# ANRGUSC/DEFER

Hardware: AMD Instinct MI355X
Metric: images/sec (whole node) ResNet50 pipeline (higher is better)
Workload: dtype bf16; 1 GPU; model=resnet50, global_batch=256, micro_batch=256, input=224x224x3 NHWC, parallelism=pp1, compression=none, hip_graphs=False, dual_rail=False, weights=random-init

## Files before the change

defer_amd/csrc/bindings.cpp:

```cpp
#include <torch/extension.h>
#include <ATen/hip/HIPContext.h>

#include <cstdlib>
#include <functional>
#include <mutex>
#include <string>
#include <unordered_map>

#include "kernels.h"

namespace {

using at::Tensor;
using defer_hip::ConvParams;

hipStream_t cur_stream() {
    return at::cuda::getCurrentHIPStream().stream();
}

const void* bptr(const Tensor& t) { return t.data_ptr(); }
void* bptr_mut(Tensor& t) { return t.data_ptr(); }

void check_bf16(const Tensor& t, const char* name) {
    TORCH_CHECK(t.is_cuda(), name, " must be on GPU");
// ... 377 lines not shown
    int64_t max_blocks) {
    check_bf16(x, "x");
    check_bf16(w3, "w3");
    check_bf16(w1, "w1");
    check_bf16(res, "res");
    TORCH_CHECK(x.dim() == 4 && w3.dim() == 4 && w1.dim() == 4 &&
                w3.size(1) == 1 && w3.size(2) == 1 && w1.size(1) == 1 &&
                w1.size(2) == 1, "conv1x1_chain wants NHWC x, 1x1 weights");
    TORCH_CHECK(mode >= 0 && mode <= 2, "mode must be 0, 1 or 2");
    int NB = x.size(0), H = x.size(1), W = x.size(2), K1 = x.size(3);
    int N1 = w3.size(0), N2 = w1.size(0);
    TORCH_CHECK(w3.size(3) == K1 && w1.size(3) == N1, "channel mismatch");
    TORCH_CHECK(res.dim() == 4 && res.size(0) == NB && res.size(1) == H &&
                res.size(2) == W && res.size(3) == N1,
                "res must match the expand output");
    TORCH_CHECK((!s3 || s3->numel() == N1) && (!b3 || b3->numel() == N1) &&
                (!s1 || s1->numel() == N2) && (!b1 || b1->numel() == N2),
                "scale/bias length must equal the conv's Cout");
    long M = (long)NB * H * W;
    TORCH_CHECK(M < (1LL << 31), "M too large");
    if (mode != 2 && K1 % 64 == 0 && N1 % 64 == 0 && N2 % 64 == 0) {
        auto y = at::empty({NB, H, W, N1}, x.options());
        auto a2 = at::empty({NB, H, W, N2}, x.options());
        if (defer_hip::launch_conv1x1_chain(
                bptr(x), bptr(w3), fptr_opt(s3, "s3", ones_buf(), N1),
                fptr_opt(b3, "b3", zeros_buf(), N1), bptr(res),
                bptr_mut(y), relu3, bptr(w1),
                fptr_opt(s1, "s1", ones_buf(), N2),
                fptr_opt(b1, "b1", zeros_buf(), N2), bptr_mut(a2), relu1,
                (int)M, K1, N1, N2, mode == 1, (int)max_blocks,
                cur_stream()))
            return {y, a2};
    }
    auto y = conv2d_bn_act(x, w3, s3, b3, res, 1, 0, relu3);
    auto a2 = conv2d_bn_act(y, w1, s1, b1, c10::nullopt, 1, 0, relu1);
    return {y, a2};
}

Tensor bn_act(Tensor x, Tensor scale, Tensor bias, bool relu) {
    if (is_f32(x, "x")) {
        check_f32(x, "x");
        int C = x.size(-1);
        TORCH_CHECK(C % 4 == 0, "fp32 bn_act needs C % 4 == 0, got ", C);
        TORCH_CHECK(scale.is_cuda() && bias.is_cuda() &&
                    scale.numel() == C && bias.numel() == C,
                    "scale/bias must be GPU tensors of length C");
        auto out = at::empty_like(x);
        auto sf = scale.to(at::kFloat).contiguous();
        auto bf = bias.to(at::kFloat).contiguous();
        defer_hip::launch_bn_act_f32(f32ptr(x), f32ptr(sf), f32ptr(bf),
                                     out.data_ptr<float>(), x.numel() / 4,
                                     C / 4, relu, cur_stream());
        return out;
    }
    check_bf16(x, "x");
    int C = x.size(-1);
    TORCH_CHECK(C % 8 == 0, "C must be a multiple of 8");
    auto out = at::empty_like(x);
    auto sf = scale.to(at::kFloat).contiguous();
    auto bf = bias.to(at::kFloat).contiguous();
    defer_hip::launch_bn_act(bptr(x), sf.data_ptr<float>(),
                             bf.data_ptr<float>(), bptr_mut(out),
                             x.numel() / 8, C / 8, relu, cur_stream());
    return out;
}

Tensor add_act(Tensor a, Tensor b, bool relu) {
    if (is_f32(a, "a")) {
        check_f32(a, "a");
        check_f32(b, "b");
        TORCH_CHECK(a.sizes() == b.sizes(), "shape mismatch");
        TORCH_CHECK(a.numel() % 4 == 0,
                    "fp32 add_act needs numel % 4 == 0");
        auto out = at::empty_like(a);
        defer_hip::launch_add_act_f32(f32ptr(a), f32ptr(b),
                                      out.data_ptr<float>(), a.numel() / 4,
                                      relu, cur_stream());
        return out;
    }
    check_bf16(a, "a");
    check_bf16(b, "b");
    TORCH_CHECK(a.sizes() == b.sizes(), "shape mismatch");
    TORCH_CHECK(a.numel() % 8 == 0, "numel must be a multiple of 8");
    auto out = at::empty_like(a);
    defer_hip::launch_add_act(bptr(a), bptr(b), bptr_mut(out),
                              a.numel() / 8, relu, cur_stream());
    return out;
}

Tensor relu(Tensor x) {
    if (is_f32(x, "x")) {
        check_f32(x, "x");
        TORCH_CHECK(x.numel() % 4 == 0, "fp32 relu needs numel % 4 == 0");
        auto out = at::empty_like(x);
        defer_hip::launch_relu_f32(f32ptr(x), out.data_ptr<float>(),
                                   x.numel() / 4, cur_stream());
        return out;
    }
    check_bf16(x, "x");
    TORCH_CHECK(x.numel() % 8 == 0, "numel must be a multiple of 8");
    auto out = at::empty_like(x);
    defer_hip::launch_relu(bptr(x), bptr_mut(out), x.numel() / 8,
                           cur_stream());
    return out;
}

Tensor softmax(Tensor x) {
    if (is_f32(x, "x")) {
        check_f32(x, "x");
        TORCH_CHECK(x.dim() >= 1 && x.numel() > 0, "softmax of nothing");
        int cols = x.size(-1);
        long rows = x.numel() / cols;
        auto out = at::empty_like(x);
        defer_hip::launch_softmax_f32(f32ptr(x), out.data_ptr<float>(),
                                      (int)rows, cols, cur_stream());
        return out;
    }
    check_bf16(x, "x");
    int cols = x.size(-1);
    long rows = x.numel() / cols;
    auto out = at::empty_like(x);
    defer_hip::launch_softmax(bptr(x), bptr_mut(out), (int)rows, cols,
                              cur_stream());
    return out;
}

Tensor maxpool2d(Tensor x, int64_t kernel, int64_t stride, int64_t pad) {
    if (is_f32(x, "x")) {
        check_f32(x, "x");
        TORCH_CHECK(x.dim() == 4, "x must be NHWC");
        int NB = x.size(0), H = x.size(1), W = x.size(2), C = x.size(3);
        TORCH_CHECK(C % 4 == 0, "fp32 maxpool2d needs C % 4 == 0, got ", C);
        int OH = (int)((H + 2 * pad - kernel) / stride + 1);
        int OW = (int)((W + 2 * pad - kernel) / stride + 1);
        auto out = at::empty({NB, OH, OW, C}, x.options());
        defer_hip::launch_maxpool_f32(f32ptr(x), out.data_ptr<float>(), NB, H,
                                 W, C, OH, OW, (int)kernel, (int)stride,
                                 (int)pad, cur_stream());
        return out;
    }
    check_bf16(x, "x");
    TORCH_CHECK(x.dim() == 4, "x must be NHWC");
    int NB = x.size(0), H = x.size(1), W = x.size(2), C = x.size(3);
    TORCH_CHECK(C % 8 == 0, "C must be a multiple of 8");
    int OH = (int)((H + 2 * pad - kernel) / stride + 1);
    int OW = (int)((W + 2 * pad - kernel) / stride + 1);
    auto out = at::empty({NB, OH, OW, C}, x.options());
    defer_hip::launch_maxpool(bptr(x), bptr_mut(out), NB, H, W, C, OH, OW,
                              (int)kernel, (int)stride, (int)pad,
                              cur_stream());
    return out;
}

Tensor avgpool2d(Tensor x, int64_t kernel, int64_t stride, int64_t pad) {
    if (is_f32(x, "x")) {
        check_f32(x, "x");
        TORCH_CHECK(x.dim() == 4, "x must be NHWC");
        int NB = x.size(0), H = x.size(1), W = x.size(2), C = x.size(3);
        TORCH_CHECK(C % 4 == 0, "fp32 avgpool2d needs C % 4 == 0, got ", C);
        int OH = (int)((H + 2 * pad - kernel) / stride + 1);
        int OW = (int)((W + 2 * pad - kernel) / stride + 1);
        auto out = at::empty({NB, OH, OW, C}, x.options());
        defer_hip::launch_avgpool_f32(f32ptr(x), out.data_ptr<float>(), NB, H,
                                 W, C, OH, OW, (int)kernel, (int)stride,
                                 (int)pad, cur_stream());
        return out;
    }
    check_bf16(x, "x");
    TORCH_CHECK(x.dim() == 4, "x must be NHWC");
    int NB = x.size(0), H = x.size(1), W = x.size(2), C = x.size(3);
    TORCH_CHECK(C % 8 == 0, "C must be a multiple of 8");
    int OH = (int)((H + 2 * pad - kernel) / stride + 1);
    int OW = (int)((W + 2 * pad - kernel) / stride + 1);
    auto out = at::empty({NB, OH, OW, C}, x.options());
    defer_hip::launch_avgpool(bptr(x), bptr_mut(out), NB, H, W, C, OH,
                              OW, (int)kernel, (int)stride, (int)pad,
                              cur_stream());
    return out;
}

Tensor concat_lastdim(std::vector<Tensor> xs) {
    TORCH_CHECK(!xs.empty(), "concat of nothing");
    auto base = xs[0].sizes().vec();
    int nd = (int)base.size();
    long rows = 1;
    for (int i = 0; i + 1 < nd; ++i) rows *= base[i];
    long ctot = 0;
    const bool f32 = is_f32(xs[0], "concat input");
    for (auto& t : xs) {
        if (f32) check_f32(t, "concat input");
        else check_bf16(t, "concat input");
        TORCH_CHECK((int)t.sizes().size() == nd, "rank mismatch");
        for (int i = 0; i + 1 < nd; ++i)
            TORCH_CHECK(t.size(i) == base[i], "leading-dim mismatch");
        ctot += t.size(nd - 1);
    }
    base[nd - 1] = ctot;
    auto out = at::empty(base, xs[0].options());
    hipStream_t s = cur_stream();
    if (f32) {
        if (xs.size() == 2 && xs[0].size(nd - 1) % 4 == 0 &&
            xs[1].size(nd - 1) % 4 == 0) {
            defer_hip::launch_cat2_f32(f32ptr(xs[0]), f32ptr(xs[1]),
                                       out.data_ptr<float>(), rows,
                                       (int)xs[0].size(nd - 1),
                                       (int)xs[1].size(nd - 1), s);
            return out;
        }
        long coff = 0;
        for (auto& t : xs) {
            long cj = t.size(nd - 1);
            hipMemcpy2DAsync((char*)bptr_mut(out) + coff * 4, ctot * 4,
                             bptr(t), cj * 4, cj * 4, rows,
                             hipMemcpyDeviceToDevice, s);
            coff += cj;
        }
        return out;
    }
    if (xs.size() == 2 && xs[0].size(nd - 1) % 8 == 0 &&
        xs[1].size(nd - 1) % 8 == 0) {
        defer_hip::launch_cat2(bptr(xs[0]), bptr(xs[1]), bptr_mut(out),
                               rows, (int)xs[0].size(nd - 1),
                               (int)xs[1].size(nd - 1), s);
        return out;
    }
    long coff = 0;
    for (auto& t : xs) {
        long cj = t.size(nd - 1);
        hipMemcpy2DAsync((char*)bptr_mut(out) + coff * 2, ctot * 2,
                         bptr(t), cj * 2, cj * 2, rows,
                         hipMemcpyDeviceToDevice, s);
        coff += cj;
    }
    return out;
}

Tensor global_avg_pool(Tensor x) {
    if (is_f32(x, "x")) {
        check_f32(x, "x");
        TORCH_CHECK(x.dim() == 4, "x must be NHWC");
        int NB = x.size(0), HW = x.size(1) * x.size(2), C = x.size(3);
        TORCH_CHECK(C % 4 == 0,
                    "fp32 global_avg_pool needs C % 4 == 0, got ", C);
        TORCH_CHECK(HW > 0, "empty spatial extent");
        auto out = at::empty({NB, C}, x.options());
        defer_hip::launch_gap_f32(f32ptr(x), out.data_ptr<float>(), NB, HW,
                                  C, cur_stream());
        return out;
    }
    check_bf16(x, "x");
    TORCH_CHECK(x.dim() == 4, "x must be NHWC");
    int NB = x.size(0), HW = x.size(1) * x.size(2), C = x.size(3);
    TORCH_CHECK(C % 8 == 0, "C must be a multiple of 8");
    auto out = at::empty({NB, C}, x.options());
    defer_hip::launch_gap(bptr(x), bptr_mut(out), NB, HW, C, cur_stream());
    return out;
}

std::tuple<int64_t, int64_t, int64_t> field_shape(const Tensor& t) {
    auto sz = t.sizes();
    int nd = sz.size();
    if (nd == 1) return {1, 1, sz[0]};
    if (nd == 2) return {1, sz[0], sz[1]};
    int64_t d0 = 1;
    for (int i = 0; i + 2 < nd; ++i) d0 *= sz[i];
    return {d0, sz[nd - 2], sz[nd - 1]};
}

Tensor zfp_encode(Tensor x, int64_t rate, c10::optional<Tensor> out,
                  int64_t phases = 3) {
    TORCH_CHECK(x.is_cuda() && x.is_contiguous(), "x must be GPU contig");
    bool bf16 = x.scalar_type() == at::kBFloat16;
    TORCH_CHECK(bf16 || x.scalar_type() == at::kFloat, "bf16/f32 only");
    auto [d0, d1, d2] = field_shape(x);
    long nb = ((d0 + 3) / 4) * ((d1 + 3) / 4) * ((d2 + 3) / 4);
    long bytes = nb * rate * 8;
    Tensor o;
    if (out) {
        TORCH_CHECK(out->numel() == bytes && out->is_contiguous()
                    && out->scalar_type() == at::kByte, "bad out buffer");
        o = *out;
    } else {
        o = at::empty({bytes},
                      x.options().dtype(at::kByte));
    }
    defer_hip::launch_zfp_encode(bptr(x), bptr_mut(o), bf16, (int)d0,
                                 (int)d1, (int)d2, (int)rate,
                                 cur_stream(), (int)phases);
    return o;
}

Tensor zfp_decode(Tensor wire, std::vector<int64_t> shape, int64_t rate,
                  bool bf16_out) {
    TORCH_CHECK(wire.is_cuda() && wire.is_contiguous()
                && wire.scalar_type() == at::kByte, "bad wire");
    auto o = at::empty(shape, wire.options().dtype(
                                  bf16_out ? at::kBFloat16 : at::kFloat));
    auto [d0, d1, d2] = field_shape(o);
    defer_hip::launch_zfp_decode(bptr(wire), bptr_mut(o), bf16_out,
                                 (int)d0, (int)d1, (int)d2, (int)rate,
                                 cur_stream());
    return o;
}

void fp8_encode(Tensor x, Tensor out) {
    check_bf16(x, "x");
    long n = x.numel();
    TORCH_CHECK(out.is_cuda() && out.is_contiguous()
                && out.scalar_type() == at::kByte
                && out.numel() == n + 4, "bad fp8 wire buffer");
    defer_hip::launch_fp8_encode(bptr(x), n, bptr_mut(out),
                                 cur_stream());
}

Tensor fp8_decode(Tensor wire, std::vector<int64_t> shape) {
    TORCH_CHECK(wire.is_cuda() && wire.is_contiguous()
                && wire.scalar_type() == at::kByte, "bad wire");
    auto y = at::empty(shape, wire.options().dtype(at::kBFloat16));
    TORCH_CHECK(y.numel() + 4 == wire.numel(), "wire/shape mismatch");
    defer_hip::launch_fp8_decode(bptr(wire), y.numel(), bptr_mut(y),
                                 cur_stream());
    return y;
}

Tensor lz4_compress(Tensor x) {
    TORCH_CHECK(x.is_cuda() && x.is_contiguous()
                && x.scalar_type() == at::kByte, "x must be GPU u8 contig");
    long n = x.numel();
    TORCH_CHECK(n > 0, "empty input");
    auto scratch = at::empty({defer_hip::lz4_scratch_bytes(n)},
                             x.options());
    auto o = at::empty({defer_hip::lz4_max_compressed(n)}, x.options());
    defer_hip::launch_lz4_compress(bptr(x), n, bptr_mut(scratch),
                                   bptr_mut(o), cur_stream());
    long nb = (n + 4095) / 4096;
    auto hdr_cpu = o.narrow(0, 4 * (2 + nb), 4).to(at::kCPU);
    uint32_t total;
    std::memcpy(&total, hdr_cpu.data_ptr(), 4);
    return o.narrow(0, 0, 4 * (2 + nb + 1) + (long)total);
}

void lz4_compress_into(Tensor x, Tensor scratch, Tensor out,
                       Tensor len_out) {
    TORCH_CHECK(x.is_cuda() && x.is_contiguous()
                && x.scalar_type() == at::kByte, "x must be GPU u8 contig");
    long n = x.numel();
    TORCH_CHECK(n > 0, "empty input");
    TORCH_CHECK(scratch.numel() >= defer_hip::lz4_scratch_bytes(n)
                && scratch.is_cuda(), "scratch too small");
    TORCH_CHECK(out.numel() >= defer_hip::lz4_max_compressed(n)
                && out.is_cuda() && out.scalar_type() == at::kByte,
                "out too small");
    TORCH_CHECK(len_out.is_cuda() && len_out.numel() == 1
                && len_out.scalar_type() == at::kLong, "bad len_out");
    hipStream_t s = cur_stream();
    defer_hip::launch_lz4_compress(bptr(x), n, bptr_mut(scratch),
                                   bptr_mut(out), s);
    defer_hip::launch_lz4_wire_len(bptr(out), n, bptr_mut(len_out), s);
}

Tensor lz4_decompress(Tensor comp, int64_t raw_len) {
    TORCH_CHECK(comp.is_cuda() && comp.is_contiguous()
                && comp.scalar_type() == at::kByte, "bad comp buffer");
    TORCH_CHECK(raw_len > 0, "raw_len must be positive");
    auto o = at::empty({raw_len}, comp.options());
    defer_hip::launch_lz4_decompress(bptr(comp), bptr_mut(o), raw_len,
                                     cur_stream());
    return o;
}

}

PYBIND11_MODULE(TORCH_EXTENSION_NAME, m) {
    m.def("conv2d_bn_act", &conv2d_bn_act, py::arg("x"), py::arg("w"),
          py::arg("scale"), py::arg("bias"), py::arg("res"),
          py::arg("stride"), py::arg("pad"), py::arg("relu"));
    m.def("linear", &linear);
    m.def("bn_act", &bn_act);
    m.def("conv1x1_prebn", &conv1x1_prebn, py::arg("x"),
          py::arg("w"), py::arg("scale"), py::arg("bias"),
          py::arg("out_scale") = py::none(),
          py::arg("out_bias") = py::none());
    m.def("conv1x1_chain", &conv1x1_chain, py::arg("x"), py::arg("w3"),
          py::arg("s3"), py::arg("b3"), py::arg("res"), py::arg("relu3"),
          py::arg("w1"), py::arg("s1"), py::arg("b1"), py::arg("relu1"),
          py::arg("mode") = 0, py::arg("max_blocks") = 0);
    m.def("add_act", &add_act);
    m.def("relu", &relu);
    m.def("softmax", &softmax);
    m.def("maxpool2d", &maxpool2d);
    m.def("avgpool2d", &avgpool2d);
    m.def("concat_lastdim", &concat_lastdim);
    m.def("global_avg_pool", &global_avg_pool);
    m.def("zfp_encode", &zfp_encode, py::arg("x"), py::arg("rate"),
          py::arg("out") = py::none(), py::arg("phases") = 3);
    m.def("zfp_decode", &zfp_decode);
    m.def("fp8_encode", &fp8_encode);
    m.def("fp8_decode", &fp8_decode);
    m.def("lz4_compress", &lz4_compress);
    m.def("lz4_compress_into", &lz4_compress_into);
    m.def("lz4_scratch_bytes",
          [](int64_t n) { return defer_hip::lz4_scratch_bytes(n); });
    m.def("lz4_decompress", &lz4_decompress);
}
```

defer_amd/csrc/kernels.h:

```cpp
#pragma once

#include <hip/hip_runtime.h>

namespace defer_hip {

struct ConvParams {
    const void* x;
    const void* w;
    const float* scale;
    const float* bias;
    const void* res;
    void* out;
    const void* zbuf;
    int M, K, Cout;
    int NB, H, W, Cin;
    int OH, OW, R, S, stride, pad;
    unsigned int owmul, ohmul, cmul, smul;
};

void launch_conv_igemm(const ConvParams& p, bool relu, bool has_res,
                       bool gemm_mode, bool stem_mode, hipStream_t s);
void launch_pad_channels(const void* x, void* y, long rows, int C, int C8,
                         hipStream_t s);
void launch_pad2d(const void* x, void* y, int NB, int H, int W, int C,
                  int PH, int PW, int ph0, int pw0, hipStream_t s);
bool launch_conv_swin(const ConvParams& p, bool relu, int R, int stride,
                      hipStream_t s);
void launch_swin_repack_w(const void* w, void* wp, int Cout, int R,
                          int C, int Kpad, hipStream_t s);
void launch_stem_repack_w(const void* w, void* wp, int Cout, int R, int S,
                          int C, int TR, hipStream_t s);

void launch_gemm_prebn(const void* x, const void* w, const float* ps,
                       const float* pb, const float* os, const float* ob,
                       const void* zbuf, void* out, int M, int K,
                       int Cout, hipStream_t s);

bool launch_conv1x1_chain(const void* x, const void* w3, const float* s3,
                          const float* b3, const void* res, void* y,
                          bool relu3, const void* w1, const float* s1,
                          const float* b1, void* a2, bool relu1, int M,
                          int K1, int N1, int N2, bool force,
                          int max_blocks, hipStream_t s);

void launch_bn_act(const void* x, const float* scale, const float* bias,
                   void* y, long total8, int c8, bool relu, hipStream_t s);
void launch_add_act(const void* a, const void* b, void* y, long total8,
                    bool relu, hipStream_t s);
void launch_relu(const void* x, void* y, long total8, hipStream_t s);
void launch_cat2(const void* a, const void* b, void* y, long rows,
                 int c1, int c2, hipStream_t s);
void launch_softmax(const void* x, void* y, int rows, int cols,
                    hipStream_t s);
void launch_maxpool(const void* x, void* y, int NB, int H, int W, int C,
                    int OH, int OW, int k, int stride, int pad,
                    hipStream_t s);
void launch_avgpool(const void* x, void* y, int NB, int H, int W, int C,
                    int OH, int OW, int k, int stride, int pad,
                    hipStream_t s);
void launch_gap(const void* x, void* y, int NB, int HW, int C,
                hipStream_t s);

struct ConvF32Params {
    const float* x;
    const float* w;
    const float* scale;
    const float* bias;
    const float* res;
    float* out;
    int M, K, Cout;
    int H, W, Cin;
    int OH, OW, S, stride, pad;
    int relu;
};
void launch_conv_f32(const ConvF32Params& p, bool gemm_mode, int tile,
                     hipStream_t s);
void launch_pad_channels_f32(const float* x, float* y, long rows, int C,
                             int C4, hipStream_t s);

void launch_bn_act_f32(const float* x, const float* scale, const float* bias,
                       float* y, long total4, int c4, bool relu,
                       hipStream_t s);
void launch_add_act_f32(const float* a, const float* b, float* y,
                        long total4, bool relu, hipStream_t s);
void launch_relu_f32(const float* x, float* y, long total4, hipStream_t s);
void launch_cat2_f32(const float* a, const float* b, float* y, long rows,
                     int c1, int c2, hipStream_t s);
void launch_softmax_f32(const float* x, float* y, int rows, int cols,
                        hipStream_t s);
void launch_maxpool_f32(const float* x, float* y, int NB, int H, int W,
                        int C, int OH, int OW, int k, int stride, int pad,
                        hipStream_t s);
void launch_avgpool_f32(const float* x, float* y, int NB, int H, int W,
                        int C, int OH, int OW, int k, int stride, int pad,
                        hipStream_t s);
void launch_gap_f32(const float* x, float* y, int NB, int HW, int C,
                    hipStream_t s);

void launch_zfp_encode(const void* x, void* out, bool bf16_in, int d0,
                       int d1, int d2, int rate, hipStream_t s,
                       int phases = 3);
void launch_zfp_decode(const void* wire, void* y, bool bf16_out, int d0,
                       int d1, int d2, int rate, hipStream_t s);

void launch_fp8_encode(const void* x, long n, void* out, hipStream_t s);
void launch_fp8_decode(const void* wire, long n, void* y, hipStream_t s);

long lz4_max_compressed(long n);
long lz4_scratch_bytes(long n);
void launch_lz4_compress(const void* in, long n, void* scratch, void* out,
                         hipStream_t s);
void launch_lz4_wire_len(const void* out_stream, long n, void* len_out,
                         hipStream_t s);
void launch_lz4_decompress(const void* comp, void* out, long raw_len,
                           hipStream_t s);

}
```

defer_amd/ops/__init__.py:

```python

import os
from typing import Optional

import torch

from defer_amd.ops import reference as _ref

_hip = None
_hip_err: Optional[Exception] = None


def _load_hip():
    global _hip, _hip_err
    if _hip is not None or _hip_err is not None:
        return _hip
    try:
        import defer_amd._hip_ops as m

        _hip = m
    except Exception as e:
        _hip_err = e
    return _hip


def hip_available() -> bool:
    return _load_hip() is not None


def _backend(x: torch.Tensor):
    if x.is_cuda:
        m = _load_hip()
        if m is None:
            raise RuntimeError(
                "defer_amd HIP extension (defer_amd._hip_ops) is not built "
                "but a GPU tensor was passed. Build it with "
                "`python -m defer_amd.build` (gfx950). Import error: "
                f"{_hip_err!r}"
            )
        return m
    return None


def conv2d_bn_act(x, w, scale=None, bias=None, stride=1, padding=1,
                  act="none", residual=None):
    m = _backend(x)
    if m is None:
        return _ref.conv2d_bn_act(x, w, scale, bias, stride, padding, act,
                                  residual)
    return m.conv2d_bn_act(x, w, scale, bias, residual, stride, padding,
                           act == "relu")


def conv1x1_prebn(x, w, scale, bias, out_scale=None, out_bias=None):
    m = _backend(x)
    if m is None:
        z = _ref.batchnorm_apply(x, scale, bias, "relu")
        y = _ref.conv2d_bn_act(z, w, None, None, 1, 0, "none", None)
        if out_scale is not None:
            y = _ref.batchnorm_apply(y, out_scale, out_bias, "relu")
        return y
    if x.dtype == torch.float32:
        z = batchnorm_apply(x, scale, bias, "relu")
        y = conv2d_bn_act(z, w, None, None, 1, 0, "none", None)
        if out_scale is not None:
            y = batchnorm_apply(y, out_scale, out_bias, "relu")
        return y
    return m.conv1x1_prebn(x, w, scale, bias, out_scale, out_bias)


_CHAIN_MODES = {None: 0, "": 0, "force": 1, "0": 2}
_chain_env = os.environ.get("DEFER_CONV_CHAIN")
if _chain_env not in _CHAIN_MODES:
    raise ValueError(
        f"DEFER_CONV_CHAIN={_chain_env!r}: expected unset, '0' or 'force'")
_CHAIN_MODE = _CHAIN_MODES[_chain_env]


def conv1x1_chain(x, w3, s3, b3, residual, act3, w1, s1, b1, act1,
                  mode=None, max_blocks=0):
    m = _backend(x)
    if m is None:
        y = _ref.conv2d_bn_act(x, w3, s3, b3, 1, 0, act3, residual)
        a2 = _ref.conv2d_bn_act(y, w1, s1, b1, 1, 0, act1, None)
        return y, a2
    if x.dtype == torch.float32:
        y = conv2d_bn_act(x, w3, s3, b3, 1, 0, act3, residual)
        a2 = conv2d_bn_act(y, w1, s1, b1, 1, 0, act1, None)
        return y, a2
    return m.conv1x1_chain(x, w3, s3, b3, residual, act3 == "relu", w1, s1,
                           b1, act1 == "relu",
                           _CHAIN_MODE if mode is None else mode, max_blocks)


def batchnorm_apply(x, scale, bias, act="none"):
    m = _backend(x)
    if m is None:
        return _ref.batchnorm_apply(x, scale, bias, act)
    return m.bn_act(x, scale, bias, act == "relu")


def add_act(a, b, act="relu"):
    m = _backend(a)
    if m is None:
        return _ref.add_act(a, b, act)
    return m.add_act(a, b, act == "relu")


def relu(x):
    m = _backend(x)
    if m is None:
        return _ref.relu(x)
    return m.relu(x)


def maxpool2d(x, kernel=3, stride=2, padding=1):
    m = _backend(x)
    if m is None:
        return _ref.maxpool2d(x, kernel, stride, padding)
    return m.maxpool2d(x, kernel, stride, padding)


def avgpool2d(x, kernel=2, stride=2, padding=0):
    m = _backend(x)
    if m is None:
        return _ref.avgpool2d(x, kernel, stride, padding)
    return m.avgpool2d(x, kernel, stride, padding)


def concat_channels(xs):
    m = _backend(xs[0])
    if m is None:
        return _ref.concat_channels(xs)
    return m.concat_lastdim(list(xs))


def global_avg_pool(x):
    m = _backend(x)
    if m is None:
        return _ref.global_avg_pool(x)
    return m.global_avg_pool(x)


def linear(x, w, bias=None):
    m = _backend(x)
    if m is None:
        return _ref.linear(x, w, bias)
    return m.linear(x, w, bias)


def softmax(x):
    m = _backend(x)
    if m is None:
        return _ref.softmax(x)
    return m.softmax(x)
```

defer_amd/parallel/fusion.py:

```python

from typing import List

import torch.nn as nn

from defer_amd.graph import GraphNode, LayerGraph
from defer_amd.models.layers import AddAct, ConvBNAct


class FusedConvAddAct(nn.Module):

    def __init__(self, conv: ConvBNAct, act: str):
        super().__init__()
        self.conv = conv
        self.act = act

    def forward(self, x, residual):
        from defer_amd import ops

        c = self.conv
        return ops.conv2d_bn_act(
            x, c.weight.to(x.dtype), c.scale, c.bias, stride=c.stride,
            padding=c.padding, act=self.act, residual=residual)


def fuse_residual_adds(graph: LayerGraph) -> LayerGraph:
    consumers = {}
    for n in graph.nodes:
        for p in n.inputs:
            consumers.setdefault(p, []).append(n.name)
    out_name = graph.output

    nodes: List[GraphNode] = []
    by_name = {n.name: n for n in graph.nodes}
    fused_away = set()
    for n in graph.nodes:
        if n.name in fused_away:
            continue
        lay = n.layer
        if isinstance(lay, AddAct):
            for idx, p in enumerate(n.inputs):
                pn = by_name.get(p)
                if (pn is not None and isinstance(pn.layer, ConvBNAct)
                        and pn.layer.act == "none"
                        and consumers.get(p, []) == [n.name]
                        and p != out_name):
                    other = n.inputs[1 - idx]
                    fused = FusedConvAddAct(pn.layer, lay.act)
                    nodes = [m for m in nodes if m.name != p]
                    nodes.append(GraphNode(n.name, fused,
                                           [pn.inputs[0], other]))
                    fused_away.add(p)
                    break
            else:
                nodes.append(n)
            continue
        nodes.append(n)
    return LayerGraph(nodes, output=graph.output)


class ChainedExpandReduce(nn.Module):

    def __init__(self, expand: FusedConvAddAct, reduce: ConvBNAct):
        super().__init__()
        self.expand = expand
        self.reduce = reduce

    def forward(self, x, residual):
        from defer_amd import ops

        c3, c1 = self.expand.conv, self.reduce
        return ops.conv1x1_chain(
            x, c3.weight.to(x.dtype), c3.scale, c3.bias, residual,
            self.expand.act, c1.weight.to(x.dtype), c1.scale, c1.bias,
            c1.act)


class _Pick(nn.Module):

    def __init__(self, index: int):
        super().__init__()
        self.index = index

    def forward(self, t):
        return t[self.index]

    def extra_repr(self):
        return f"item {self.index}"


def _is_pointwise(c: ConvBNAct) -> bool:
    return c.kernel == 1 and c.stride == 1 and c.padding == 0


def fuse_expand_reduce(graph: LayerGraph) -> LayerGraph:
    consumers = {}
    for n in graph.nodes:
        for p in n.inputs:
            consumers.setdefault(p, []).append(n)

    partner = {}
    for n in graph.nodes:
        if not (isinstance(n.layer, FusedConvAddAct)
                and _is_pointwise(n.layer.conv)):
            continue
        for c in consumers.get(n.name, []):
            if (isinstance(c.layer, ConvBNAct) and _is_pointwise(c.layer)
                    and c.inputs == [n.name] and not c.kwargs):
                partner[n.name] = c
                break
    taken = {c.name for c in partner.values()}

    nodes: List[GraphNode] = []
    for n in graph.nodes:
        if n.name in taken:
            continue
        c = partner.get(n.name)
        if c is None:
            nodes.append(n)
            continue
        pair = n.name + "__chain"
        nodes.append(GraphNode(pair, ChainedExpandReduce(n.layer, c.layer),
                               list(n.inputs), dict(n.kwargs)))
        nodes.append(GraphNode(n.name, _Pick(0), [pair]))
        nodes.append(GraphNode(c.name, _Pick(1), [pair]))
    return LayerGraph(nodes, output=graph.output)
```

defer_amd/parallel/pipeline.py:

```python

import queue
import threading
import time
from dataclasses import dataclass
from typing import Callable, List, Optional

import torch
import torch.distributed as dist

from defer_amd.config import PipelineConfig
from defer_amd.graph import GraphModel
from defer_amd.parallel.comm import (Codec, DualRailRing, HopForwarder,
                                     P2PRing, dtype_bytes, dual_active,
                                     dual_bw_boost, hop_via, make_ring,
                                     split_point)
from defer_amd.parallel.partitioner import (as_graph_model, auto_partition,
                                            partition_model)



@dataclass
class StageStats:
    items: int = 0
    images: int = 0
    compute_s: float = 0.0
    compute_ms: float = 0.0
    bytes_in: int = 0
    bytes_out: int = 0
    bytes_fwd: int = 0


class StageExecutor:

    _capture_lock = threading.Lock()

    def __init__(self, stage: GraphModel, device, dtype: torch.dtype,
                 use_graph: bool = False, fuse: bool = True,
                 chain: bool = True):
        if fuse:
            from defer_amd.parallel.fusion import (fuse_expand_reduce,
                                                   fuse_residual_adds)

            g = fuse_residual_adds(stage.graph)
            if chain:
                g = fuse_expand_reduce(g)
            stage = GraphModel(g, name=stage.model_name)
        self.model = stage
        self.device = torch.device(device)
        self.dtype = dtype
        self.use_graph = use_graph and self.device.type == "cuda"
        stage.to(self.device)
        if self.device.type == "cuda":
            for p in stage.parameters():
                if p.dim() >= 2:
                    p.data = p.data.to(dtype).contiguous()
                else:
                    p.data = p.data.float()
        self._graph = None
        self._static_in = None
        self._static_out = None

    def _capture(self, x: torch.Tensor):
        self._static_in = x.clone()
        torch.cuda.synchronize()
        s = torch.cuda.Stream()
        with torch.cuda.stream(s):
            self.model(self._static_in)
        torch.cuda.current_stream().wait_stream(s)
        torch.cuda.synchronize()
        g = torch.cuda.CUDAGraph()
        with torch.cuda.graph(g):
            self._static_out = self.model(self._static_in)
        self._graph = g

    def run(self, x: torch.Tensor) -> torch.Tensor:
        if not self.use_graph:
            with torch.no_grad():
                return self.model(x)
        if self._graph is None:
            try:
                with StageExecutor._capture_lock:
                    self._capture(x)
            except Exception:
                self.use_graph = False
                with torch.no_grad():
                    return self.model(x)
        self._static_in.copy_(x)
        self._graph.replay()
        return self._static_out

    def output_shape(self, input_shape) -> tuple:
        was = self.use_graph
        self.use_graph = False
        try:
            with torch.no_grad():
                x = torch.zeros(*input_shape, device=self.device,
                                dtype=self.dtype
                                if self.device.type == "cuda"
                                else torch.float32)
                return tuple(self.run(x).shape)
        finally:
            self.use_graph = was



class DEFER:

    def __init__(self, computeNodes: List, config: Optional[PipelineConfig] = None):
        self.computeNodes = list(computeNodes)
        self.cfg = config or PipelineConfig()
        self.stats: List[StageStats] = []

    def run_defer(self, model, partition_layers: Optional[List[str]],
                  input_stream: "queue.Queue", output_stream: "queue.Queue"):
        cfg = self.cfg
        n = len(self.computeNodes)
        if partition_layers is None and cfg.weights_dir and n > 1:
            from defer_amd import checkpoint

            mani = checkpoint.load_manifest(cfg.weights_dir)
            if mani["num_stages"] != n:
                raise ValueError(
                    f"checkpoint has {mani['num_stages']} stages but "
                    f"{n} compute nodes were given")
            partition_layers = list(mani["cut_points"])
        if partition_layers is None:
            from defer_amd.parallel.calibrate import find_calibration

            gm0 = as_graph_model(model)
            partition_layers, stages = auto_partition(
                gm0, n,
                input_shape=tuple(cfg.input_shape)
                if cfg.input_shape else (1, 224, 224, 3),
                measured_us=find_calibration(gm0.model_name,
                                             cfg.calibration_file))
        else:
            stages = partition_model(model, partition_layers)
        if len(stages) != n:
            raise ValueError(
                f"{len(stages)} stages for {n} compute nodes")
        if cfg.partition_dump_dir:
            from defer_amd.utils.visualize import dump_partition

            dump_partition(stages, cfg.partition_dump_dir,
                           cut_points=partition_layers)
        if cfg.weights_dir:
            from defer_amd import checkpoint

            for i, s in enumerate(stages):
                checkpoint.load_stage(s, cfg.weights_dir, i)
        dtype = cfg.torch_dtype()
        execs = [StageExecutor(s, dev, dtype, cfg.use_hip_graphs)
                 for s, dev in zip(stages, self.computeNodes)]
        self.stats = [StageStats() for _ in range(n)]
        self.errors: List = [None] * n
        qs = [input_stream] + [queue.Queue(cfg.ring_depth)
                               for _ in range(n)]
        ready = [threading.Event() for _ in range(n)]

        def worker(i: int):
            ex = execs[i]
            dev = ex.device
            if dev.type == "cuda":
                torch.cuda.set_device(dev)
            ready[i].set()
            st = self.stats[i]
            while True:
                x = qs[i].get()
                if x is None:
                    qs[i + 1].put(None)
                    return
                try:
                    if dev.type == "cuda":
                        x = x.to(dev, dtype, non_blocking=True)
                    t0 = time.perf_counter()
                    with torch.no_grad():
                        y = ex.run(x)
                    st.compute_s += time.perf_counter() - t0
                except Exception as e:
                    self.errors[i] = e
                    qs[i + 1].put(None)
                    while qs[i].get() is not None:
                        pass
                    return
                st.items += 1
                st.images += x.shape[0] if x.dim() > 1 else 1
                qs[i + 1].put(y)

        threads = [threading.Thread(target=worker, args=(i,), daemon=True)
                   for i in range(n)]
        for t in threads:
            t.start()
        for e in ready:
            e.wait()

        while True:
            y = qs[n].get()
            if y is None:
# ... 308 lines not shown
```

setup.py:

```python

import os
from pathlib import Path

from setuptools import setup

os.environ.setdefault("PYTORCH_ROCM_ARCH", "gfx950")

from torch.utils.cpp_extension import BuildExtension, CUDAExtension

ROOT = Path(__file__).parent
CSRC = ROOT / "defer_amd" / "csrc"

sources = [str(CSRC / f) for f in
           ["bindings.cpp", "conv.hip", "prebn.hip", "chain.hip", "elementwise.hip", "pool.hip",
            "codec.hip", "lz4.hip", "conv_f32.hip", "ops_f32.hip"]
           if (CSRC / f).exists()]

setup(
    name="defer_amd",
    version="0.1.0",
    packages=["defer_amd"],
    ext_modules=[
        CUDAExtension(
            name="defer_amd._hip_ops",
            sources=sources,
            extra_compile_args={
                "cxx": ["-O3", "-std=c++17"],
                "nvcc": ["-O3", "-std=c++17", "--offload-arch=gfx950"],
            },
        )
    ],
    cmdclass={"build_ext": BuildExtension},
)
```

Measured before the change: 48080 images/sec.

## Fuse ResNet stem 7x7 conv, BN, ReLU and 3x3 maxpool into one kernel

Adds a dedicated HIP kernel that computes the stem 7x7 stride-2 conv with MFMA, applies BN and ReLU, and keeps conv output rows in an LDS ring buffer so the 3x3 stride-2 maxpool runs in place. Input rows are streamed through a shared ring in row bands per image, and staging of the next rows overlaps with the MFMA compute. A graph pass replaces the ConvBNAct+MaxPool pair with the fused node. This avoids writing and re-reading the large 112x112x64 intermediate activation and saves a kernel launch, at the cost of a specialised kernel with high register and LDS use that may limit occupancy.

```diff
diff --git a/defer_amd/csrc/bindings.cpp b/defer_amd/csrc/bindings.cpp
--- a/defer_amd/csrc/bindings.cpp
+++ b/defer_amd/csrc/bindings.cpp
@@ -553,6 +553,84 @@
     return out;
 }
 
+struct StemPoolStats {
+    std::mutex mu;
+    int64_t launches = 0;
+    int64_t bands = 0, rows_per_band = 0;
+};
+StemPoolStats& stem_pool_stats_ref() {
+    static StemPoolStats st;
+    return st;
+}
+
+py::dict stem_pool_stats() {
+    auto& st = stem_pool_stats_ref();
+    std::lock_guard<std::mutex> g(st.mu);
+    py::dict d;
+    d["launches"] = st.launches;
+    d["bands"] = st.bands;
+    d["rows_per_band"] = st.rows_per_band;
+    return d;
+}
+
+Tensor conv_bn_act_maxpool(Tensor x, Tensor w, c10::optional<Tensor> scale,
+                           c10::optional<Tensor> bias, int64_t stride,
+                           int64_t pad, bool relu, int64_t pool_kernel,
+                           int64_t pool_stride, int64_t pool_pad,
+                           int64_t mode, int64_t max_blocks) {
+    check_bf16(x, "x");
+    check_bf16(w, "w");
+    TORCH_CHECK(x.dim() == 4, "x must be NHWC");
+    TORCH_CHECK(w.dim() == 4, "w must be OHWI");
+    TORCH_CHECK(mode >= 0 && mode <= 2, "mode must be 0, 1 or 2");
+    TORCH_CHECK(max_blocks >= 0, "max_blocks must be >= 0");
+    int NB = x.size(0), H = x.size(1), W = x.size(2), Cin = x.size(3);
+    int Cout = w.size(0), R = w.size(1), S = w.size(2);
+    TORCH_CHECK(w.size(3) == Cin, "w Cin mismatch");
+    TORCH_CHECK((!scale || scale->numel() == Cout) &&
+                (!bias || bias->numel() == Cout),
+                "scale/bias length must equal Cout");
+    int OH = (int)((H + 2 * pad - R) / stride + 1);
+    int OW = (int)((W + 2 * pad - S) / stride + 1);
+    if (mode != 2 && NB > 0 && OH > 0 && OW > 0 &&
+        (long)NB * OH * OW < (1LL << 31) &&
+        defer_hip::stem_pool_supported(Cin, Cout, R, S, (int)stride,
+                                       (int)pad, relu, (int)pool_kernel,
+                                       (int)pool_stride, (int)pool_pad,
+                                       OH, OW)) {
+        hipStream_t s = cur_stream();
+        const int TR = 24, Keff = R * TR;
+        auto wp = cached_weight_prep(w, TR, [&] {
+            auto t = at::empty({Cout, Keff}, w.options());
+            defer_hip::launch_stem_repack_w(bptr(w), bptr_mut(t), Cout, R,
+                                            S, Cin, TR, s);
+            return t;
+        });
+        int POH = (OH + 2 - 3) / 2 + 1, POW = (OW + 2 - 3) / 2 + 1;
+        auto out = at::empty({NB, POH, POW, Cout}, x.options());
+        defer_hip::StemPoolParams q{};
+        q.x = bptr(x);
+        q.wp = bptr(wp);
+        q.scale = fptr_opt(scale, "scale", ones_buf(), Cout);
+        q.bias = fptr_opt(bias, "bias", zeros_buf(), Cout);
+        q.out = bptr_mut(out);
+        q.NB = NB; q.H = H; q.W = W;
+        q.OH = OH; q.OW = OW; q.POH = POH; q.POW = POW;
+        auto used = defer_hip::launch_stem_pool(q, (int)max_blocks, s);
+        {
+            auto& st = stem_pool_stats_ref();
+            std::lock_guard<std::mutex> g(st.mu);
+            ++st.launches;
+            st.bands = used.bands;
+            st.rows_per_band = used.rpb;
+        }
+        return out;
+    }
+    auto y = conv2d_bn_act(x, w, scale, bias, c10::nullopt, stride, pad,
+                           relu);
+    return maxpool2d(y, pool_kernel, pool_stride, pool_pad);
+}
+
 Tensor avgpool2d(Tensor x, int64_t kernel, int64_t stride, int64_t pad) {
     if (is_f32(x, "x")) {
         check_f32(x, "x");
@@ -786,6 +864,13 @@
           py::arg("s3"), py::arg("b3"), py::arg("res"), py::arg("relu3"),
           py::arg("w1"), py::arg("s1"), py::arg("b1"), py::arg("relu1"),
           py::arg("mode") = 0, py::arg("max_blocks") = 0);
+    m.def("conv_bn_act_maxpool", &conv_bn_act_maxpool, py::arg("x"),
+          py::arg("w"), py::arg("scale"), py::arg("bias"),
+          py::arg("stride"), py::arg("pad"), py::arg("relu"),
+          py::arg("pool_kernel"), py::arg("pool_stride"),
+          py::arg("pool_pad"), py::arg("mode") = 0,
+          py::arg("max_blocks") = 0);
+    m.def("stem_pool_stats", &stem_pool_stats);
     m.def("add_act", &add_act);
     m.def("relu", &relu);
     m.def("softmax", &softmax);
diff --git a/defer_amd/csrc/kernels.h b/defer_amd/csrc/kernels.h
--- a/defer_amd/csrc/kernels.h
+++ b/defer_amd/csrc/kernels.h
@@ -42,6 +42,23 @@
                           const float* b1, void* a2, bool relu1, int M,
                           int K1, int N1, int N2, bool force,
                           int max_blocks, hipStream_t s);
+
+struct StemPoolParams {
+    const void* x;
+    const void* wp;
+    const float* scale;
+    const float* bias;
+    void* out;
+    int NB, H, W;
+    int OH, OW;
+    int POH, POW;
+    int bands, rpb;
+};
+bool stem_pool_supported(int Cin, int Cout, int R, int S, int stride,
+                         int pad, bool relu, int pk, int ps, int pp,
+                         int OH, int OW);
+StemPoolParams launch_stem_pool(const StemPoolParams& p, int max_blocks,
+                                hipStream_t s);
 
 void launch_bn_act(const void* x, const float* scale, const float* bias,
                    void* y, long total8, int c8, bool relu, hipStream_t s);
diff --git a/defer_amd/csrc/stem_pool.hip b/defer_amd/csrc/stem_pool.hip
--- /dev/null
+++ b/defer_amd/csrc/stem_pool.hip
@@ -0,0 +1,227 @@
+#include "common.h"
+#include "kernels.h"
+
+using defer_hip::StemPoolParams;
+
+#define SP_TPB 256
+#define SP_NW (SP_TPB / WAVE)
+#define SP_MAXOW 128
+#define SP_C 64
+#define SP_KS 6
+#define SP_TR 24
+#define SP_K (7 * SP_TR)
+#define SP_IR 16
+#define SP_PITCH 792
+#define SP_SROWS 4
+#define SP_SPT ((SP_PITCH + SP_TPB - 1) / SP_TPB)
+
+__global__ __launch_bounds__(SP_TPB, 2) void stem_pool_kernel(
+    StemPoolParams p) {
+    const bf16* __restrict__ X = (const bf16*)p.x;
+    const bf16* __restrict__ Wp = (const bf16*)p.wp;
+    bf16* __restrict__ OUT = (bf16*)p.out;
+
+    __shared__ __attribute__((aligned(16)))
+    bf16 ring[3 * SP_MAXOW * SP_C];
+    __shared__ __attribute__((aligned(16)))
+    bf16 inr[SP_IR * SP_PITCH];
+
+    const int tid = threadIdx.x;
+    const int wave = __builtin_amdgcn_readfirstlane(tid / WAVE);
+    const int lane = tid % WAVE;
+    const int lo16 = lane & 15;
+    const int hi4 = lane >> 4;
+
+    bf16x8 bfr[4][SP_KS];
+    float sc[4], bi[4];
+#pragma unroll
+    for (int ni = 0; ni < 4; ++ni) {
+        const int n = ni * 16 + lo16;
+        sc[ni] = p.scale[n];
+        bi[ni] = p.bias[n];
+#pragma unroll
+        for (int ks = 0; ks < SP_KS; ++ks) {
+            const int k = ks * 32 + hi4 * 8;
+            bf16x8 z = {0, 0, 0, 0, 0, 0, 0, 0};
+            bfr[ni][ks] = (k < SP_K) ? load_bf16x8(Wp + n * SP_K + k) : z;
+        }
+    }
+
+    int kr[SP_KS], kt[SP_KS];
+#pragma unroll
+    for (int ks = 0; ks < SP_KS; ++ks) {
+        const int k = ks * 32 + hi4 * 8;
+        kr[ks] = k / SP_TR;
+        kt[ks] = k % SP_TR;
+    }
+
+    const int MF = (p.OW + 15) / 16;
+    const int LEN = 6 * (p.OW - 1) + SP_TR;
+    const int W3 = p.W * 3;
+    const int items = p.NB * p.bands;
+
+    bf16 sv[SP_SROWS][SP_SPT];
+    auto stage_load = [&](const bf16* xn, int pa, int n) {
+#pragma unroll
+        for (int i = 0; i < SP_SROWS; ++i) {
+            const int ih = pa + i - 3;
+            const bool rowok = i < n && ih >= 0 && ih < p.H;
+            const bf16* src = xn + (long)(rowok ? ih : 0) * W3;
+#pragma unroll
+            for (int j = 0; j < SP_SPT; ++j) {
+                const int e = tid + j * SP_TPB - 9;
+                sv[i][j] = (rowok && e >= 0 && e < W3) ? src[e] : (bf16)0.f;
+            }
+        }
+    };
+    auto stage_store = [&](int pa, int n) {
+#pragma unroll
+        for (int i = 0; i < SP_SROWS; ++i) {
+            if (i >= n) continue;
+            bf16* dst = inr + ((pa + i) & (SP_IR - 1)) * SP_PITCH;
+#pragma unroll
+            for (int j = 0; j < SP_SPT; ++j) {
+                const int e = tid + j * SP_TPB;
+                if (e < LEN) dst[e] = sv[i][j];
+            }
+        }
+    };
+
+    auto compute = [&](int r0, int t) {
+        const int dr = t >= MF ? 1 : 0;
+        const int mf = t - dr * MF;
+        int colA = mf * 16 + lo16;
+        if (colA >= p.OW) colA = p.OW - 1;
+        const int prow = 2 * (r0 + dr);
+        bf16x8 a[SP_KS];
+#pragma unroll
+        for (int ks = 0; ks < SP_KS; ++ks) {
+            const void* q = __builtin_assume_aligned(
+                inr + ((prow + kr[ks]) & (SP_IR - 1)) * SP_PITCH +
+                    colA * 6 + kt[ks], 4);
+            __builtin_memcpy(&a[ks], q, 16);
+        }
+        f32x4 acc[4];
+#pragma unroll
+        for (int ni = 0; ni < 4; ++ni) acc[ni] = {0.f, 0.f, 0.f, 0.f};
+#pragma unroll
+        for (int ks = 0; ks < SP_KS; ++ks)
+#pragma unroll
+            for (int ni = 0; ni < 4; ++ni)
+                acc[ni] = MFMA_BF16_16x16x32(a[ks], bfr[ni][ks], acc[ni]);
+        bf16* row = ring + ((r0 + dr) % 3) * (SP_MAXOW * SP_C);
+#pragma unroll
+        for (int e = 0; e < 4; ++e) {
+            const int col = mf * 16 + hi4 * 4 + e;
+#pragma unroll
+            for (int ni = 0; ni < 4; ++ni) {
+                const int c = (ni * 16 + lo16) ^ (hi4 << 4);
+                float v = acc[ni][e] * sc[ni] + bi[ni];
+                row[col * SP_C + c] = f2bf(apply_act(v, ACT_RELU));
+            }
+        }
+    };
+
+    for (int item = blockIdx.x; item < items; item += gridDim.x) {
+        const int nb = item / p.bands;
+        const int band = item - nb * p.bands;
+        const int p0 = band * p.rpb;
+        const int p1 = min(p0 + p.rpb, p.POH);
+        const bf16* xn = X + (long)nb * p.H * W3;
+
+        const int s_first = p0 > 0 ? -1 : 0;
+        const int s_end = p1 - p0;
+        auto step_r0 = [&](int s) { return s < 0 ? 2 * p0 - 1 : 2 * (p0 + s); };
+        auto step_nr = [&](int s) {
+            return s < 0 ? 1 : min(2, p.OH - step_r0(s));
+        };
+        auto step_hi = [&](int s) {
+            return 2 * (step_r0(s) + step_nr(s) - 1) + 8;
+        };
+
+        int staged = 2 * step_r0(s_first);
+        for (const int hi = step_hi(s_first); staged < hi;
+             staged += SP_SROWS) {
+            const int n = min(SP_SROWS, hi - staged);
+            stage_load(xn, staged, n);
+            stage_store(staged, n);
+        }
+        staged = step_hi(s_first);
+        asm volatile("s_waitcnt lgkmcnt(0)" ::: "memory");
+        __builtin_amdgcn_s_barrier();
+
+        for (int s = s_first; s < s_end; ++s) {
+            const int r0 = step_r0(s);
+            const int nt = step_nr(s) * MF;
+            const int nhi = s + 1 < s_end ? step_hi(s + 1) : staged;
+            const int nnew = nhi - staged;
+            stage_load(xn, staged, nnew);
+#pragma unroll 1
+            for (int t = wave; t < nt; t += SP_NW) compute(r0, t);
+            stage_store(staged, nnew);
+            staged = nhi;
+            asm volatile("s_waitcnt lgkmcnt(0)" ::: "memory");
+            __builtin_amdgcn_s_barrier();
+            if (s >= 0) {
+                const int pr = p0 + s;
+                bf16* orow = OUT + ((long)nb * p.POH + pr) * p.POW * SP_C;
+#pragma unroll 1
+                for (int i = tid; i < p.POW * 8; i += SP_TPB) {
+                    const int q = i >> 3, c8 = i & 7;
+                    s16x8 best;
+#pragma unroll
+                    for (int dr = -1; dr <= 1; ++dr) {
+                        int r = 2 * pr + dr;
+                        if (r < 0 || r >= p.OH) r = 2 * pr;
+                        const bf16* row =
+                            ring + (r % 3) * (SP_MAXOW * SP_C);
+#pragma unroll
+                        for (int dc = -1; dc <= 1; ++dc) {
+                            int c = 2 * q + dc;
+                            if (c < 0 || c >= p.OW) c = 2 * q;
+                            const s16x8 v = __builtin_bit_cast(
+                                s16x8,
+                                load_bf16x8(
+                                    row + c * SP_C +
+                                    ((c8 * 8) ^ (((c >> 2) & 3) << 4))));
+                            best = (dr == -1 && dc == -1)
+                                       ? v
+                                       : __builtin_elementwise_max(best, v);
+                        }
+                    }
+                    const bf16x8 o = __builtin_bit_cast(bf16x8, best);
+                    store_bf16x8(orow + q * SP_C + c8 * 8, o);
+                }
+                asm volatile("s_waitcnt lgkmcnt(0)" ::: "memory");
+                __builtin_amdgcn_s_barrier();
+            }
+        }
+    }
+}
+
+namespace defer_hip {
+
+bool stem_pool_supported(int Cin, int Cout, int R, int S, int stride,
+                         int pad, bool relu, int pk, int ps, int pp,
+                         int OH, int OW) {
+    return Cin == 3 && Cout == SP_C && R == 7 && S == 7 && stride == 2 &&
+           pad == 3 && relu && pk == 3 && ps == 2 && pp == 1 && OH >= 1 &&
+           OW >= 1 && OW <= SP_MAXOW;
+}
+
+StemPoolParams launch_stem_pool(const StemPoolParams& p0, int max_blocks,
+                                hipStream_t s) {
+    StemPoolParams p = p0;
+    int bands = (512 + p.NB - 1) / p.NB;
+    if (bands > p.POH) bands = p.POH;
+    if (bands < 1) bands = 1;
+    p.rpb = (p.POH + bands - 1) / bands;
+    p.bands = (p.POH + p.rpb - 1) / p.rpb;
+    long items = (long)p.NB * p.bands;
+    int grid = (int)(items < 512 ? items : 512);
+    if (max_blocks > 0 && grid > max_blocks) grid = max_blocks;
+    hipLaunchKernelGGL(stem_pool_kernel, dim3(grid), dim3(SP_TPB), 0, s, p);
+    return p;
+}
+
+}
diff --git a/defer_amd/ops/__init__.py b/defer_amd/ops/__init__.py
--- a/defer_amd/ops/__init__.py
+++ b/defer_amd/ops/__init__.py
@@ -92,6 +92,41 @@
                            _CHAIN_MODE if mode is None else mode, max_blocks)
 
 
+_STEM_POOL_MODES = {None: 0, "": 0, "force": 1, "0": 2}
+_stem_pool_env = os.environ.get("DEFER_STEM_POOL")
+if _stem_pool_env not in _STEM_POOL_MODES:
+    raise ValueError(
+        f"DEFER_STEM_POOL={_stem_pool_env!r}: expected unset, '0' or 'force'")
+_STEM_POOL_MODE = _STEM_POOL_MODES[_stem_pool_env]
+
+
+def conv_bn_act_maxpool(x, w, scale, bias, stride, padding, act,
+                        pool_kernel, pool_stride, pool_padding, mode=None,
+                        max_blocks=0):
+    m = _backend(x)
+    if m is None:
+        y = _ref.conv2d_bn_act(x, w, scale, bias, stride, padding, act, None)
+        return _ref.maxpool2d(y, pool_kernel, pool_stride, pool_padding)
+    if x.dtype == torch.float32:
+        y = conv2d_bn_act(x, w, scale, bias, stride, padding, act, None)
+        return maxpool2d(y, pool_kernel, pool_stride, pool_padding)
+    if act not in ("relu", "none"):
+        raise ValueError(f"act={act!r}: expected 'relu' or 'none'")
+    return m.conv_bn_act_maxpool(x, w, scale, bias, stride, padding,
+                                 act == "relu", pool_kernel, pool_stride,
+                                 pool_padding,
+                                 _STEM_POOL_MODE if mode is None else mode,
+                                 max_blocks)
+
+
+def stem_pool_stats():
+    m = _load_hip()
+    if m is None:
+        raise RuntimeError(
+            f"defer_amd HIP extension is not built: {_hip_err!r}")
+    return dict(m.stem_pool_stats())
+
+
 def batchnorm_apply(x, scale, bias, act="none"):
     m = _backend(x)
     if m is None:
diff --git a/defer_amd/parallel/fusion.py b/defer_amd/parallel/fusion.py
--- a/defer_amd/parallel/fusion.py
+++ b/defer_amd/parallel/fusion.py
@@ -4,7 +4,7 @@
 import torch.nn as nn
 
 from defer_amd.graph import GraphNode, LayerGraph
-from defer_amd.models.layers import AddAct, ConvBNAct
+from defer_amd.models.layers import AddAct, ConvBNAct, MaxPool
 
 
 class FusedConvAddAct(nn.Module):
@@ -124,3 +124,58 @@
         nodes.append(GraphNode(n.name, _Pick(0), [pair]))
         nodes.append(GraphNode(c.name, _Pick(1), [pair]))
     return LayerGraph(nodes, output=graph.output)
+
+
+class FusedConvPool(nn.Module):
+
+    def __init__(self, conv: ConvBNAct, pool: MaxPool):
+        super().__init__()
+        self.conv = conv
+        self.pool = pool
+
+    def forward(self, x):
+        from defer_amd import ops
+
+        c, q = self.conv, self.pool
+        return ops.conv_bn_act_maxpool(
+            x, c.weight.to(x.dtype), c.scale, c.bias, c.stride, c.padding,
+            c.act, q.kernel, q.stride, q.padding)
+
+
+def _is_stem_pool(c: ConvBNAct, q: MaxPool) -> bool:
+    return (c.cin == 3 and c.cout == 64 and c.kernel == 7 and c.stride == 2
+            and c.padding == 3 and c.act == "relu"
+            and (q.kernel, q.stride, q.padding) == (3, 2, 1))
+
+
+def fuse_conv_pool(graph: LayerGraph) -> LayerGraph:
+    consumers = {}
+    for n in graph.nodes:
+        for p in n.inputs:
+            consumers.setdefault(p, []).append(n)
+
+    partner = {}
+    for n in graph.nodes:
+        if not (type(n.layer) is ConvBNAct and len(n.inputs) == 1
+                and not n.kwargs and n.name != graph.output):
+            continue
+        cs = consumers.get(n.name, [])
+        if (len(cs) == 1 and type(cs[0].layer) is MaxPool
+                and cs[0].inputs == [n.name] and not cs[0].kwargs
+                and _is_stem_pool(n.layer, cs[0].layer)):
+            partner[n.name] = cs[0]
+    pools = {q.name: c for c, q in partner.items()}
+
+    by_name = {n.name: n for n in graph.nodes}
+    nodes: List[GraphNode] = []
+    for n in graph.nodes:
+        if n.name in partner:
+            continue
+        c = pools.get(n.name)
+        if c is None:
+            nodes.append(n)
+            continue
+        conv = by_name[c]
+        nodes.append(GraphNode(n.name, FusedConvPool(conv.layer, n.layer),
+                               list(conv.inputs)))
+    return LayerGraph(nodes, output=graph.output)
diff --git a/defer_amd/parallel/pipeline.py b/defer_amd/parallel/pipeline.py
--- a/defer_amd/parallel/pipeline.py
+++ b/defer_amd/parallel/pipeline.py
@@ -38,12 +38,14 @@
                  use_graph: bool = False, fuse: bool = True,
                  chain: bool = True):
         if fuse:
-            from defer_amd.parallel.fusion import (fuse_expand_reduce,
+            from defer_amd.parallel.fusion import (fuse_conv_pool,
+                                                   fuse_expand_reduce,
                                                    fuse_residual_adds)
 
             g = fuse_residual_adds(stage.graph)
             if chain:
                 g = fuse_expand_reduce(g)
+            g = fuse_conv_pool(g)
             stage = GraphModel(g, name=stage.model_name)
         self.model = stage
         self.device = torch.device(device)
diff --git a/setup.py b/setup.py
--- a/setup.py
+++ b/setup.py
@@ -12,7 +12,7 @@
 CSRC = ROOT / "defer_amd" / "csrc"
 
 sources = [str(CSRC / f) for f in
-           ["bindings.cpp", "conv.hip", "prebn.hip", "chain.hip", "elementwise.hip", "pool.hip",
+           ["bindings.cpp", "conv.hip", "prebn.hip", "chain.hip", "stem_pool.hip", "elementwise.hip", "pool.hip",
             "codec.hip", "lz4.hip", "conv_f32.hip", "ops_f32.hip"]
            if (CSRC / f).exists()]
 
```

Result: faster. 51640 images/sec (median of 6 runs) (+7.4%).
